# microsoft/fadtk

Measured on AMD Instinct MI355X. Metric: FAD scores/sec + cov-GEMM TFLOP/s (% MFMA peak), N=100k D=512, higher is better.
Workload: dtype f16 in, f16 MFMA with f32 accumulate over <= 8192-row runs, f64 across runs (moments); split-f16 MFMA iterations (f32 accumulate) + exact int8-MFMA products (int32 accumulate) + f64 correction (Frechet)

## Files before the change

### fadtk_amd/csrc/frechet.hip

```cpp
#include "frechet_internal.h"
#include "ns_mean.h"
#include "ns_fast.h"
#include "ns_fast_big.h"
#include "ns_fast_res.h"

#include <algorithm>
#include <atomic>
#include <cmath>
#include <type_traits>

namespace fad {

Pool& thread_pool(int device) {
    static thread_local PerThreadDevice<Pool> set;
    return set.get(device);
}
Workspace* free_slot(int device) {
    Pool& p = thread_pool(device);
    for (Workspace& w : p.slot)
        if (!w.busy) { w.pool = &p; return &w; }
    return nullptr;
}

SongKnobs SongKnobs::from_env() {
// ... 582 lines not shown
    int k = 1, upto = resident ? 1 : 9;
    for (;;) {
        for (; k < upto; ++k) {
            const int cur = k & 1;
            nsf::SplitArgs g = split_args();
            g.A[0] = Z[cur]; g.B[0] = Y[cur]; g.C[0] = T; g.alpha = -0.5f; g.beta_eye = 1.5f; g.gamma = 1.0f;
            g.partials = partials; g.skip = &s32_0->done; g.k = k;
            if (big) FAD_TRY(fast_split_big(d, nsf::SP_T, g, st, (unsigned)B, device));
            else fast_split(d, nsf::SP_T, g, st, (unsigned)B);
            g = split_args();
            g.A[0] = Y[cur]; g.B[0] = T; g.C[0] = Y[cur ^ 1]; g.A[1] = T; g.B[1] = Z[cur]; g.C[1] = Z[cur ^ 1];
            g.skip = &s32_0->upd_skip[k & 1];
            g.k = k; g.max_low = kMaxLow; g.nslots = big ? fast_big_t_slots(d, (unsigned)B) : nb * nb; g.chk_partials = partials; g.thr_pred = pred_threshold(ws.pool, d);
            if (big) FAD_TRY(fast_split_big(d, nsf::SP_U, g, st, (unsigned)B, device));
            else fast_split(d, nsf::SP_U, g, st, (unsigned)B);
        }
        if (!res_full) {
            nsf::DigArgs dg;
            memset(&dg, 0, sizeof(dg));
            dg.d = d; dg.gen = gen; dg.hA = hdr_b; dg.hB = reinterpret_cast<nsf::MatHdr*>(at(L.hdr)); dg.pstride = (int64_t)L.stride; dg.s32 = s32_0;
            dg.Y[0] = Y[0]; dg.Y[1] = Y[1]; dg.dig[0] = digY[0]; dg.dig[1] = digY[1]; dg.dig_t[0] = digYt[0]; dg.dig_t[1] = digYt[1];
            hipLaunchKernelGGL(nsf::nsf_digitize, dim3((unsigned)((dd / 16 + 255) / 256), 2, (unsigned)B), dim3(256), 0, st, dg);
        }
        if (!res_full) {
            nsf::I8Args a;
            memset(&a, 0, sizeof(a));
            a.Adig = digY[0]; a.Bdig = digYt[0]; a.Adig_alt = digY[1]; a.Bdig_alt = digYt[1]; a.sel = &s32_0->final_iter;
            a.d = d; a.gen = gen; a.hA = hdr_b; a.hB = reinterpret_cast<nsf::MatHdr*>(at(L.hdr)); a.pstride = (int64_t)L.stride; a.hstride = (int64_t)hs;
            a.skip = &s32_0->skip_corr; a.stats = h_stats; a.st = st0; a.A64in = A64;
            a.Y[0] = Y[0]; a.Y[1] = Y[1]; a.Z[0] = Z[0]; a.Z[1] = Z[1]; a.s32 = s32_0; a.host_words = h_words; a.host_vals = h_vals;
            for (int64_t b = 0; b < B; ++b) reinterpret_cast<int*>(reinterpret_cast<char*>(h_words) + b * hs)[12] = 0;
            if (big && d >= 256) FAD_TRY(fast_i8_big(d, nsf::I8_G, a, st, (unsigned)B, device));
            else fast_i8(d, nsf::I8_G, a, st, (unsigned)B);
        }
        FAD_HIP_TRY(hipGetLastError());
        FAD_HIP_TRY(hipStreamSynchronize(st));
        bool pending = false;
        for (int64_t b = 0; b < B; ++b) {
            if (settled[b]) continue;
            const int* hw = reinterpret_cast<const int*>(reinterpret_cast<const char*>(h_words) + b * hs);
            const double* hv = reinterpret_cast<const double*>(reinterpret_cast<const char*>(h_vals) + b * hs);
            const double* hx = reinterpret_cast<const double*>(reinterpret_cast<const char*>(h_stats) + b * hs);
            if (hw[12] != gen) return set_error(FAD_ERR_HIP, "the correction kernel of the batched fast chain left no result for song %lld", (long long)b);
            MixedResult r;
            fast_decide_one(hw, hv, hx, nb, &r);
            if (r.status == 0 && k < kMaxLow && !resident) { pending = true; continue; }
            settled[b] = 1;
            if (r.status == 1) { ok[b] = 1; tr_sqrt[b] = std::sqrt(r.c) * r.tr_scaled; }
            if (trace)
                fprintf(stderr, "[fad fast songs] song %lld: status %d iters %d decided_at %d res %.3e est %.3e tr %.6e c %.3e (words bad %d done %d ok %d failed %d skipped %d)\n",
                        (long long)b, r.status, r.iters, r.decided_at, r.res, r.est, r.tr_scaled, r.c, hw[0], hw[1], hw[5], hw[6], hw[11]);
            if (trace && b == 0) {
                fprintf(stderr, "[fad fast songs] song 0 residuals:");
                for (int q = 1; q < 16 && q <= r.iters; ++q) fprintf(stderr, " %.3e", hv[4 + q]);
                fprintf(stderr, "\n");
            }
        }
        if (!pending) break;
        upto = kMaxLow;
    }
    return FAD_OK;
}


struct PairBlock {
    size_t hdrA, hdrB, st, s32, partials, stats, A64, P, Y[2], Z[2], T, digA, digB, digY[2], digYt[2], mus, covs, Rv, Pv, Ev, stride;
};
static PairBlock pair_block(int d) {
    const size_t dd = (size_t)d * d, nb = (size_t)d / 32;
    PairBlock b; size_t o = 0;
    auto take = [&](size_t bytes) { const size_t at = o; o += (bytes + 255) & ~(size_t)255; return at; };
    b.hdrA = take(sizeof(nsf::MatHdr)); b.hdrB = take(sizeof(nsf::MatHdr)); b.st = take(sizeof(NsState)); b.s32 = take(sizeof(Ns32State));
    b.partials = take(nb * nb * sizeof(double)); b.stats = take(nsf::kTileStats * nb * nb * sizeof(double));
    b.A64 = take(8 * dd); b.P = take(8 * dd);
    b.Y[0] = take(8 * dd); b.Y[1] = take(8 * dd); b.Z[0] = take(8 * dd); b.Z[1] = take(8 * dd); b.T = take(8 * dd);
    b.digA = take(6 * dd); b.digB = take(6 * dd);
    b.digY[0] = take(6 * dd); b.digYt[0] = take(6 * dd); b.digY[1] = take(6 * dd); b.digYt[1] = take(6 * dd);
    b.mus = take(2 * (size_t)d * sizeof(double)); b.covs = take(2 * dd * sizeof(double));
    b.Rv = take(8 * dd); b.Pv = take(8 * dd); b.Ev = take(8 * dd);
    b.stride = o;
    return b;
}

static int pairs_verify_enqueue(Workspace& ws, int d, int B, hipStream_t st) {
    const size_t dd = (size_t)d * d;
    const PairBlock L = pair_block(d);
    const size_t hs = song_host_stride(d);
    char* blk = static_cast<char*>(ws.fast_pairs.p);
    char* hpin = static_cast<char*>(ws.fast_pairs_pin);
    auto at = [&](size_t off) { return blk + off; };
    auto mat = [&](size_t off) { nsf::SplitMat m; m.a = reinterpret_cast<uint4*>(at(off)); m.at = reinterpret_cast<uint4*>(at(off + 4 * dd)); return m; };
    nsf::SplitArgs g;
    memset(&g, 0, sizeof(g));
    g.d = d; g.gen = ws.multi.gen; g.hA = reinterpret_cast<nsf::MatHdr*>(at(L.hdrA)); g.hB = reinterpret_cast<nsf::MatHdr*>(at(L.hdrB));
    g.pstride = (int64_t)L.stride; g.astride = (int64_t)L.stride;
    g.st = reinterpret_cast<NsState*>(at(L.st)); g.s32 = reinterpret_cast<Ns32State*>(at(L.s32));
    const nsf::SplitMat Y[2] = {mat(L.Y[0]), mat(L.Y[1])}, Z[2] = {mat(L.Z[0]), mat(L.Z[1])};
    const int nb = d / 32;
    int* h_words = reinterpret_cast<int*>(hpin + (nsf::kHostVals + (size_t)(nsf::kTileStats + 2) * nb * nb) * sizeof(double));
    double* h_vstats = reinterpret_cast<double*>(hpin + host_vstats_off(d));
    for (int b = 0; b < B; ++b) reinterpret_cast<int*>(reinterpret_cast<char*>(h_words) + (size_t)b * hs)[13] = 0;
    fast_verify_launch(d, (unsigned)B, g, Y, Z, mat(L.Rv), mat(L.Pv), mat(L.Ev), g.s32, h_vstats, h_words, (int64_t)hs, st);
    FAD_HIP_TRY(hipGetLastError());
    FAD_HIP_TRY(hipEventRecord(ws.done_ev, st));
    return FAD_OK;
}

static int pairs_enqueue(Workspace& ws, int d, int B, const fad_moments_t* const* h1, const fad_moments_t* const* h2, int ddof,
                         int mean_dtype, hipStream_t st) {
    const size_t dd = (size_t)d * d;
    const int nb = d / 32;
    constexpr int kPairsBigMin = 3;
    const bool big = B >= kPairsBigMin && d >= 256;
    const bool wide = wide_enabled(ws.pool);
    const int max_low = wide ? kMaxLowWide : kMaxLow;
    const int device = ws.job.device;
    const PairBlock L = pair_block(d);
    const size_t hs = song_host_stride(d);
    void* const before = ws.fast_pairs.p;
    FAD_TRY(ws.fast_pairs.reserve((size_t)(B > 16 ? kMaxMultiPairs : B > 8 ? 16 : B > 4 ? 8 : 4) * L.stride + 256));
    if (!ws.fast_pairs_pin || ws.fast_pairs_pin_cap < (size_t)B * hs) {
        if (ws.fast_pairs_pin) (void)hipHostFree(ws.fast_pairs_pin);
        ws.fast_pairs_pin = nullptr; ws.fast_pairs_pin_cap = 0;
        FAD_HIP_TRY(hipHostMalloc(&ws.fast_pairs_pin, (size_t)kMaxMultiPairs * hs + 4096, hipHostMallocDefault));
        ws.fast_pairs_pin_cap = (size_t)kMaxMultiPairs * hs + 4096;
    }
    char* blk = static_cast<char*>(ws.fast_pairs.p);
    char* hpin = static_cast<char*>(ws.fast_pairs_pin);
    double* h_vals = reinterpret_cast<double*>(hpin);
    double* h_stats = h_vals + nsf::kHostVals;
    int* h_words = reinterpret_cast<int*>(h_stats + (size_t)(nsf::kTileStats + 2) * nb * nb);
    auto at = [&](size_t off) { return blk + off; };
    auto mat = [&](size_t off) { nsf::SplitMat m; m.a = reinterpret_cast<uint4*>(at(off)); m.at = reinterpret_cast<uint4*>(at(off + 4 * dd)); return m; };
    const int gen = ++ws.fast_gen;
    if (ws.fast_gen > (1 << 30)) ws.fast_gen = 1;
    ws.multi.gen = gen;
    if (ws.fast_pairs.p != before) {
        FAD_HIP_TRY(hipMemset2DAsync(at(L.hdrA), L.stride, 0, sizeof(nsf::MatHdr), (size_t)B, st));
        FAD_HIP_TRY(hipMemset2DAsync(at(L.hdrB), L.stride, 0, sizeof(nsf::MatHdr), (size_t)B, st));
    }
    nsf::MatHdr* hA = reinterpret_cast<nsf::MatHdr*>(at(L.hdrA));
    nsf::MatHdr* hB = reinterpret_cast<nsf::MatHdr*>(at(L.hdrB));
    NsState* st0 = reinterpret_cast<NsState*>(at(L.st));
    Ns32State* s32_0 = reinterpret_cast<Ns32State*>(at(L.s32));
    double* partials = reinterpret_cast<double*>(at(L.partials));
    double* stats = reinterpret_cast<double*>(at(L.stats));
    double* A64 = reinterpret_cast<double*>(at(L.A64));
    const nsf::SplitMat P = mat(L.P), Y[2] = {mat(L.Y[0]), mat(L.Y[1])}, Z[2] = {mat(L.Z[0]), mat(L.Z[1])}, T = mat(L.T);
    uint4* digY[2] = {reinterpret_cast<uint4*>(at(L.digY[0])), reinterpret_cast<uint4*>(at(L.digY[1]))};
    uint4* digYt[2] = {reinterpret_cast<uint4*>(at(L.digYt[0])), reinterpret_cast<uint4*>(at(L.digYt[1]))};

    static_assert(2 * kMaxMultiPairs <= nsf::kPrepMaxSets, "PrepArgs holds two sets per pair of a batch");
    nsf::PrepArgs pa;
    memset(&pa, 0, sizeof(pa));
    for (int b = 0; b < B; ++b) {
        pa.accs[2 * b] = moments_packed(h1[b]); pa.accs[2 * b + 1] = moments_packed(h2[b]);
        pa.runs[2 * b] = moments_runsum(h1[b]); pa.runs[2 * b + 1] = moments_runsum(h2[b]);
    }
    pa.acc[0] = pa.accs[0]; pa.acc[1] = pa.accs[1];
    pa.d = d; pa.ddof = ddof; pa.gen = gen; pa.mean_dtype = mean_dtype;
    pa.mus = reinterpret_cast<double*>(at(L.mus)); pa.covs = reinterpret_cast<double*>(at(L.covs));
    pa.dig[0] = reinterpret_cast<uint4*>(at(L.digA)); pa.dig[1] = reinterpret_cast<uint4*>(at(L.digB));
    pa.st = st0; pa.hdr[0] = hA; pa.hdr[1] = hB;
    pa.batch = 2; pa.pstride = (int64_t)L.stride; pa.no_covs = 1;
    pa.per = ((dd / 2048) % 4 == 0) ? 4 : 2;
    hipLaunchKernelGGL(nsf::nsf_prepare, dim3((unsigned)(dd / 2048 / pa.per + 1), (unsigned)(2 * B)), dim3(512), 0, st, pa);

    auto split_args = [&]() {
        nsf::SplitArgs g;
        memset(&g, 0, sizeof(g));
        g.d = d; g.gen = gen; g.hA = hA; g.hB = hB; g.pstride = (int64_t)L.stride; g.astride = (int64_t)L.stride;
        g.st = st0; g.s32 = s32_0;
        if (wide) { g.scaled = 1; g.lp_wide = 1; g.l0_scale = kWideL0Scale; g.l0_min = kWideL0Min; }
        return g;
    };
    {
        nsf::I8Args a;
        memset(&a, 0, sizeof(a));
        a.Adig = reinterpret_cast<uint4*>(at(L.digA)); a.Bdig = reinterpret_cast<uint4*>(at(L.digB)); a.d = d; a.gen = gen; a.hA = hA; a.hB = hB;
        a.pstride = (int64_t)L.stride; a.astride = (int64_t)L.stride; a.stats = stats; a.A64 = A64; a.P = P; a.st = st0;
        if (big) FAD_TRY(fast_i8_big(d, nsf::I8_A, a, st, (unsigned)B, device));
        else fast_i8(d, nsf::I8_A, a, st, (unsigned)B);
        nsf::SplitArgs g = split_args();
        g.A[0] = P; g.B[0] = P; g.C[0] = Y[1]; g.C[1] = Z[1]; g.A64 = A64; g.statsA = stats;
        if (big) FAD_TRY(fast_split_big(d, nsf::SP_FIRST, g, st, (unsigned)B, device));
        else { g.Cdig[0] = digY[1]; g.Cdig_t[0] = digYt[1]; fast_split(d, nsf::SP_FIRST, g, st, (unsigned)B); }
    }
    int want = ws.pool ? ws.pool->lp_iters : 5;
    if (want < 2) want = 2;
    if (want > max_low) want = max_low;
    for (int k = 1; k < want; ++k) {
        const int cur = k & 1;
        nsf::SplitArgs g = split_args();
        g.A[0] = Z[cur]; g.B[0] = Y[cur]; g.C[0] = T; g.alpha = -0.5f; g.beta_eye = 1.5f; g.gamma = 1.0f;
        g.partials = partials; g.skip = &s32_0->done; g.k = k;
        if (big) FAD_TRY(fast_split_big(d, nsf::SP_T, g, st, (unsigned)B, device));
        else fast_split(d, nsf::SP_T, g, st, (unsigned)B);
        g = split_args();
        g.A[0] = Y[cur]; g.B[0] = T; g.C[0] = Y[cur ^ 1]; g.A[1] = T; g.B[1] = Z[cur]; g.C[1] = Z[cur ^ 1];
        if (!big) { g.Cdig[0] = digY[cur ^ 1]; g.Cdig_t[0] = digYt[cur ^ 1]; }
        g.skip = &s32_0->upd_skip[k & 1];
        g.k = k; g.max_low = max_low; g.nslots = big ? fast_big_t_slots(d, (unsigned)B) : nb * nb; g.chk_partials = partials; g.thr_pred = pred_threshold(ws.pool, d);
        if (big) FAD_TRY(fast_split_big(d, nsf::SP_U, g, st, (unsigned)B, device));
        else fast_split(d, nsf::SP_U, g, st, (unsigned)B);
    }
    if (big) {
        nsf::DigArgs dg;
        memset(&dg, 0, sizeof(dg));
        dg.d = d; dg.gen = gen; dg.hA = hA; dg.hB = hB; dg.pstride = (int64_t)L.stride; dg.astride = (int64_t)L.stride; dg.s32 = s32_0;
        dg.Y[0] = Y[0]; dg.Y[1] = Y[1]; dg.dig[0] = digY[0]; dg.dig[1] = digY[1]; dg.dig_t[0] = digYt[0]; dg.dig_t[1] = digYt[1];
        hipLaunchKernelGGL(nsf::nsf_digitize, dim3((unsigned)((dd / 16 + 255) / 256), 2, (unsigned)B), dim3(256), 0, st, dg);
    }
    {
        nsf::I8Args a;
        memset(&a, 0, sizeof(a));
        a.Adig = digY[0]; a.Bdig = digYt[0]; a.Adig_alt = digY[1]; a.Bdig_alt = digYt[1]; a.sel = &s32_0->final_iter;
        a.d = d; a.gen = gen; a.hA = hA; a.hB = hB; a.pstride = (int64_t)L.stride; a.astride = (int64_t)L.stride; a.hstride = (int64_t)hs;
        a.skip = &s32_0->skip_corr; a.stats = h_stats; a.st = st0; a.A64in = A64;
        a.Y[0] = Y[0]; a.Y[1] = Y[1]; a.Z[0] = Z[0]; a.Z[1] = Z[1]; a.s32 = s32_0; a.host_words = h_words; a.host_vals = h_vals;
        if (wide) { a.Rv = mat(L.Rv); a.scaled = 1; }
        for (int b = 0; b < B; ++b) { int* w = reinterpret_cast<int*>(reinterpret_cast<char*>(h_words) + (size_t)b * hs); w[12] = 0; w[13] = 0; }
        if (big) FAD_TRY(fast_i8_big(d, nsf::I8_G, a, st, (unsigned)B, device));
        else fast_i8(d, nsf::I8_G, a, st, (unsigned)B);
    }
    FAD_HIP_TRY(hipGetLastError());
    if (!ws.done_ev) FAD_HIP_TRY(hipEventCreateWithFlags(&ws.done_ev, hipEventDisableTiming));
    if (wide && ws.pool && ws.pool->lp_verify) return pairs_verify_enqueue(ws, d, B, st);
    FAD_HIP_TRY(hipEventRecord(ws.done_ev, st));
    return FAD_OK;
}

static int mixed_begin(const NsProblem& pb, int device, hipStream_t stream, Workspace& ws) {
    const int d = pb.d;
    const int64_t dd = (int64_t)d * d;
    FAD_TRY(ws.mats.reserve((size_t)(6 * dd) * sizeof(double)));
    FAD_TRY(ws.mats32.reserve((size_t)(5 * dd) * sizeof(float)));
    const size_t hbytes = ws.job.fast ? fast_pinned_bytes(d) : sizeof(NsState) + sizeof(MixedResult);
    if (!ws.pinned || ws.pinned_cap < hbytes) {
        if (ws.pinned) (void)hipHostFree(ws.pinned);
        ws.pinned = nullptr; ws.pinned_cap = 0;
        FAD_HIP_TRY(hipHostMalloc(&ws.pinned, hbytes + 4096, hipHostMallocDefault));
        ws.pinned_cap = hbytes + 4096;
    }
    MixedBufs m = mixed_bufs(ws, d);
    m.hres->status = -1;
    ws.job.d = d; ws.job.device = device; ws.job.stream = stream; ws.job.k = 0;
    if (ws.job.fast) {
        ws.job.mu1 = pb.mu1; ws.job.mu2 = pb.mu2; ws.job.mean_dtype = pb.mean_dtype;
        int want = ws.pool ? ws.pool->lp_iters : 5;
        if (want < 2) want = 2;
        if (want > max_low_of(ws)) want = max_low_of(ws);
        if (ws.pool && ws.pool->lp_hopeless) want = 1;
        return fast_enqueue(ws, want);
    }
    NsProductExt ext;
    memset(&ext, 0, sizeof(ext));
    ext.stats = m.tilestats; ext.mu1 = pb.mu1; ext.mu2 = pb.mu2; ext.mean_dtype = pb.mean_dtype; ext.st = m.dstate;
    FAD_TRY(gemm_f64_product_stats_launch(d, pb.cov1, pb.cov2, m.A, &m.dstate->done, ext, stream));
    enqueue_ns_prepare(m.tilestats, d, (int)m.nb, pb.mu1, 0, pb.mu2, 0, pb.mean_dtype, m.dstate, 1, m.s32, 1, stream);
    int want = ws.pool ? ws.pool->lp_iters : 5;
    if (want < 2) want = 2;
    if (want > kMaxLow) want = kMaxLow;
    return mixed_enqueue(ws, want);
}

static int mixed_finish(Workspace& ws, MixedResult* res) {
    MixedBufs m = mixed_bufs(ws, ws.job.d);
    const int max_low = max_low_of(ws);
    bool asked = false;
    for (;;) {
        FAD_HIP_TRY(hipEventSynchronize(ws.done_ev));
        if (ws.job.fast) FAD_TRY(fast_decide(ws));
        if (m.hres->status == 5) {
            if (asked) { m.hres->status = 2; break; }
            asked = true;
            FAD_TRY(fast_verify_enqueue(ws));
            continue;
        }
        if (m.hres->status == 4) {
            ws.job.k = m.hres->iters;
            m.hres->status = 0;
        } else if (m.hres->status != 0 || ws.job.k >= max_low) {
            break;
        }
        if (ws.job.k >= max_low) break;
        const int step = (ws.job.fast && max_low > kMaxLow) ? 4 : 2;
        const int upto = (ws.job.k + step < max_low) ? ws.job.k + step : max_low;
        FAD_TRY(ws.job.fast ? fast_enqueue(ws, upto) : mixed_enqueue(ws, upto));
    }
    *res = *m.hres;
    if (res->status == 0) res->status = 2;
    if (res->status == 1 && res->decided_at >= 0 && ws.pool) ws.pool->lp_iters = res->decided_at + 1;
    if (ws.pool && ws.job.fast) {
        ws.pool->lp_hopeless = res->status == 2 && res->iters < 0;
        ws.pool->lp_verify = res->status == 1 && res->pad == 1;
    }
    return FAD_OK;
}

static bool mixed_eligible(Workspace& ws, int d, int max_iter, double tol) {
    Pool* p = ws.pool;
    if (p && p->mixed < 0) { const char* e = getenv("FAD_FRECHET_MIXED"); p->mixed = (e && e[0] == '0') ? 0 : 1; }
    return (!p || p->mixed) && d % 64 == 0 && max_iter <= 0 && tol <= 0.0;
}

static int frechet_single(int d, const double* cov1, const double* cov2, const double* mu1, const double* mu2,
                          double eps, int max_iter, double tol, int mean_dtype, int device, hipStream_t stream,
// ... 188 lines not shown
        if (moments_dim(h1[b]) != d || moments_dim(h2[b]) != d)
            return set_error(FAD_ERR_SHAPE, "Training and test covariances have different dimensions (pair %d: %d vs %d, pair 0: %d)", b,
                             moments_dim(h1[b]), moments_dim(h2[b]), d);
        if (moments_device(h1[b]) != device || moments_device(h2[b]) != device) return set_error(FAD_ERR_INVALID, "handles live on different devices");
    }
    DeviceGuard g(device);
    hipStream_t st = static_cast<hipStream_t>(stream);
    Workspace* wsp = free_slot(device);
    if (!wsp) return set_error(FAD_ERR_INVALID, "all %d Frechet slots of this thread are in flight: collect one with fad_frechet_end", Pool::kSlots);
    Workspace& ws = *wsp;
    ws.pool = &thread_pool(device);
    ws.job = Workspace::Job();
    ws.job.d = d; ws.job.device = device; ws.job.stream = st; ws.job.eps = eps; ws.job.mean_dtype = mean_dtype; ws.job.ddof = ddof;
    ws.multi = Workspace::Multi();
    ws.multi.count = count;
    for (int b = 0; b < count; ++b) { ws.multi.h1[b] = h1[b]; ws.multi.h2[b] = h2[b]; }
    if (fast_eligible(ws, d, 0, 0.0)) {
        for (int b = 0; b < count; ++b) { FAD_TRY(moments_settle(h1[b], st)); FAD_TRY(moments_settle(h2[b], st)); }
        FAD_TRY(pairs_enqueue(ws, d, count, h1, h2, ddof, mean_dtype, st));
        for (int b = 0; b < count; ++b) { FAD_TRY(moments_mark_read(h1[b], st)); FAD_TRY(moments_mark_read(h2[b], st)); }
        ws.multi.enqueued = true;
    }
    ws.busy = true;
    *job = reinterpret_cast<fad_frechet_job_t*>(wsp);
    return FAD_OK;
}

int fad_frechet_multi_end(fad_frechet_job_t* job, int count, double* out_fad, fad_diag_t* diag) {
    if (!job || !out_fad) return set_error(FAD_ERR_INVALID, "NULL argument");
    Workspace& ws = *reinterpret_cast<Workspace*>(job);
    if (!ws.busy) return set_error(FAD_ERR_INVALID, "this job was collected already");
    if (count != ws.multi.count) return set_error(FAD_ERR_INVALID, "this job holds %d pairs, not %d", ws.multi.count, count);
    const Workspace::Job j = ws.job;
    const Workspace::Multi m = ws.multi;
    DeviceGuard g(j.device);
    const int d = j.d, nb = d / 32;
    bool done[kMaxMultiPairs] = {false};
    int chain_status[kMaxMultiPairs];
    for (int b = 0; b < kMaxMultiPairs; ++b) chain_status[b] = -1;
    int rc = FAD_OK;
    if (m.enqueued) {
        const hipError_t e = hipEventSynchronize(ws.done_ev);
        if (e != hipSuccess) { ws.busy = false; return set_error(FAD_ERR_HIP, "hipEventSynchronize failed: %s", hipGetErrorString(e)); }
        const size_t hs = song_host_stride(d);
        const char* hpin = static_cast<const char*>(ws.fast_pairs_pin);
        const size_t off_stats = nsf::kHostVals * sizeof(double), off_words = off_stats + (size_t)(nsf::kTileStats + 2) * nb * nb * sizeof(double);
        const size_t off_vstats = host_vstats_off(d);
        const bool wide = wide_enabled(ws.pool);
        int learnt = -1;
        bool any_verified = false;
        for (int round = 0; round < 2; ++round) {
            bool ask = false;
            for (int b = 0; b < count; ++b) {
                if (done[b]) continue;
                const double* hv = reinterpret_cast<const double*>(hpin + (size_t)b * hs);
                const double* hx = reinterpret_cast<const double*>(hpin + (size_t)b * hs + off_stats);
                const int* hw = reinterpret_cast<const int*>(hpin + (size_t)b * hs + off_words);
                const double* hvx = reinterpret_cast<const double*>(hpin + (size_t)b * hs + off_vstats);
                if (hw[12] != m.gen) continue;
                MixedResult r;
                fast_decide_one(hw, hv, hx, nb, &r, wide ? hvx : nullptr, m.gen, wide ? kMaxLowWide : kMaxLow);
                chain_status[b] = r.status;
                if (r.too_few0 || r.too_few1) {
                    if (rc == FAD_OK) rc = set_error(FAD_ERR_TOO_FEW_ROWS, "FAD requires at least two embedding window frames in each set");
                    out_fad[b] = NAN; done[b] = true;
                    continue;
                }
                if (r.status == 5 && round == 0) { ask = true; continue; }
                if (r.status != 1) continue;
                const double tr_sqrt = sqrt(r.c) * r.tr_scaled;
                out_fad[b] = r.mean_term + r.tr1 + r.tr2 - 2.0 * tr_sqrt;
                if (diag) {
                    fad_diag_t& q = diag[b];
                    memset(&q, 0, sizeof(q));
                    q.iters = r.iters + 1; q.converged = 3; q.used_eps = 0; q.route = 2;
                    q.residual = r.res; q.scale = r.c; q.mean_term = r.mean_term; q.tr1 = r.tr1; q.tr2 = r.tr2; q.tr_sqrt = tr_sqrt;
                    q.verified = r.pad == 1 ? 1 : 0;
                }
                if (r.decided_at + 1 > learnt) learnt = r.decided_at + 1;
                if (r.pad == 1) any_verified = true;
                done[b] = true;
            }
            if (!ask) break;
            const int rv = pairs_verify_enqueue(ws, d, count, j.stream);
            if (rv != FAD_OK) { if (rc == FAD_OK) rc = rv; break; }
            const hipError_t e2 = hipEventSynchronize(ws.done_ev);
            if (e2 != hipSuccess) { ws.busy = false; return set_error(FAD_ERR_HIP, "hipEventSynchronize failed: %s", hipGetErrorString(e2)); }
        }
        if (learnt > 0 && ws.pool) ws.pool->lp_iters = learnt;
        if (ws.pool && wide) ws.pool->lp_verify = any_verified;

        int declined = 0;
        for (int b = 0; b < count; ++b) if (!done[b] && chain_status[b] == 2) ++declined;
        if (rc == FAD_OK && declined >= 2) {
            const PairBlock L = pair_block(d);
            const size_t dd = (size_t)d * d;
            char* blk = static_cast<char*>(ws.fast_pairs.p);
            const int64_t stride = (int64_t)(L.stride / sizeof(double));
            const double* mus = reinterpret_cast<const double*>(blk + L.mus);
            const double* covs = reinterpret_cast<const double*>(blk + L.covs);
            int r2 = ws.small.reserve(ns_small_bytes(d, count));
            NsState* hst = nullptr;
            if (r2 == FAD_OK) {
                NsState* dstates = static_cast<NsState*>(ws.small.p);
                enqueue_clear_states(dstates, count, j.stream);
                uint32_t mask = 0;
                for (int b = 0; b < count; ++b) if (done[b] || chain_status[b] != 2) mask |= (1u << b);
                if (mask) enqueue_mark_states_done(dstates, mask, count, j.stream);
                nsf::PrepArgs pc;
                memset(&pc, 0, sizeof(pc));
                for (int b = 0; b < count; ++b) { pc.accs[2 * b] = moments_packed(m.h1[b]); pc.accs[2 * b + 1] = moments_packed(m.h2[b]); }
                pc.d = d; pc.ddof = j.ddof; pc.batch = 2; pc.pstride = (int64_t)L.stride;
                pc.covs = reinterpret_cast<double*>(blk + L.covs);
                hipLaunchKernelGGL(nsf::nsf_pairs_covs, dim3((unsigned)(dd / 2048), (unsigned)(2 * count)), dim3(512), 0, j.stream, pc);
                NsProblem pb{d, count, covs, stride, covs + dd, stride, mus, stride, mus + d, stride, j.mean_dtype};
                r2 = run_ns(pb, 0, 0.0, j.device, j.stream, ws, &hst, false, nullptr, (ws.pool && ws.pool->f64_iters_multi > 0) ? ws.pool->f64_iters_multi + 1 : 0);
            }
            if (r2 == FAD_OK && hst) {
                int most = 0;
                for (int b = 0; b < count; ++b) {
                    if (done[b] || chain_status[b] != 2) continue;
                    const NsState& q = hst[b];
                    if (q.nonfinite || q.conv == 0 || !q.finished || q.final_iter < 0) continue;
                    const double tr_sqrt = sqrt(q.c) * q.tr_last;
                    out_fad[b] = q.mean_term + q.tr1 + q.tr2 - 2.0 * tr_sqrt;
                    if (diag) {
                        fad_diag_t& g2 = diag[b];
                        memset(&g2, 0, sizeof(g2));
                        g2.iters = q.final_iter + 1; g2.converged = q.conv; g2.used_eps = 0; g2.route = 0; g2.residual = q.res_last;
                        g2.scale = q.c; g2.mean_term = q.mean_term; g2.tr1 = q.tr1; g2.tr2 = q.tr2; g2.tr_sqrt = tr_sqrt;
                    }
                    if (q.final_iter + 1 > most) most = q.final_iter + 1;
                    done[b] = true;
                }
                if (most > 0 && ws.pool) ws.pool->f64_iters_multi = most;
            }
        }
    }
    ws.busy = false;
    ws.multi = Workspace::Multi();
    for (int b = 0; b < count; ++b) {
        if (done[b]) continue;
        const int r1 = fad_frechet_from_moments(m.h1[b], m.h2[b], j.ddof, j.eps, 0, 0.0, j.mean_dtype, j.stream, &out_fad[b], diag ? &diag[b] : nullptr);
        if (r1 != FAD_OK && rc == FAD_OK) rc = r1;
    }
    return rc;
}

int fad_frechet_cancel(fad_frechet_job_t* job) {
    if (!job) return set_error(FAD_ERR_INVALID, "NULL argument");
    Workspace& ws = *reinterpret_cast<Workspace*>(job);
    if (!ws.busy) return FAD_OK;
    DeviceGuard g(ws.job.device);
    if ((ws.job.mixed || ws.multi.enqueued) && ws.done_ev) FAD_HIP_TRY(hipEventSynchronize(ws.done_ev));
    else FAD_HIP_TRY(hipStreamSynchronize(ws.job.stream));
    ws.busy = false;
    ws.job = Workspace::Job();
    ws.multi = Workspace::Multi();
    return FAD_OK;
}

}
```

### fadtk_amd/csrc/frechet_internal.h

```cpp
#pragma once
#include "fad_common.h"
#include "ns_check.h"
#include "ns32.h"

#include <cstdlib>
#include <vector>

struct fad_moments;
namespace fad {
const double* moments_packed(const fad_moments* h);
int moments_settle(const fad_moments* h, hipStream_t st);
int moments_mark_read(const fad_moments* h, hipStream_t st);
int moments_device(const fad_moments* h);
int moments_dim(const fad_moments* h);
const float* moments_runsum(const fad_moments* h);

constexpr int kStatScal = 8;
static inline int64_t stat_blocks(int d) { return cdiv(d, 32); }
static inline size_t stat_doubles(int d) { const int64_t nb = stat_blocks(d); return (size_t)(2 * nb * d + kStatScal * nb * nb); }

constexpr int kMaxMultiPairs = 32;

struct Workspace : NsWorkspace {
    DevBuf rows, offs, songbuf, songmat, rows2, songrun, songjobs;
    DevBuf base_root;
    void* song_pin = nullptr; size_t song_pin_cap = 0;
    DevBuf mats32;
    DevBuf fast;
    int fast_gen = 0;
    DevBuf songcov;
    DevBuf fast_songs;
    void* fast_songs_pin = nullptr; size_t fast_songs_pin_cap = 0;
    DevBuf fast_pairs;
    void* fast_pairs_pin = nullptr; size_t fast_pairs_pin_cap = 0;
    struct Multi {
        int count = 0, gen = 0;
        bool enqueued = false;
        const fad_moments_t* h1[kMaxMultiPairs] = {nullptr}; const fad_moments_t* h2[kMaxMultiPairs] = {nullptr};
    } multi;
    bool busy = false;
    struct Job {
        int d = 0, device = 0, k = 0, mean_dtype = -1, ddof = 1;
        bool mixed = false;
        bool fast = false;
        int gen = 0;
        double eps = 0.0;
        hipStream_t stream = nullptr;
        const double *cov1 = nullptr, *cov2 = nullptr, *mu1 = nullptr, *mu2 = nullptr;
    } job;
    hipEvent_t done_ev = nullptr;
    struct Pool* pool = nullptr;
    void release_all() {
        release(); rows.release(); offs.release(); songbuf.release(); songmat.release(); rows2.release(); songrun.release(); songjobs.release(); mats32.release(); base_root.release(); fast.release();
        fast_songs.release(); songcov.release(); fast_pairs.release();
        if (fast_pairs_pin) { (void)hipHostFree(fast_pairs_pin); fast_pairs_pin = nullptr; fast_pairs_pin_cap = 0; }
        if (fast_songs_pin) { (void)hipHostFree(fast_songs_pin); fast_songs_pin = nullptr; fast_songs_pin_cap = 0; }
        if (done_ev) { (void)hipEventDestroy(done_ev); done_ev = nullptr; }
        if (song_pin) { (void)hipHostFree(song_pin); song_pin = nullptr; song_pin_cap = 0; }
    }
    int reserve_song_pin(size_t bytes) {
        if (song_pin && song_pin_cap >= bytes) return FAD_OK;
        if (song_pin) (void)hipHostFree(song_pin);
        song_pin = nullptr; song_pin_cap = 0;
        FAD_HIP_TRY(hipHostMalloc(&song_pin, bytes + bytes / 2 + 4096, hipHostMallocDefault));
        song_pin_cap = bytes + bytes / 2 + 4096;
        return FAD_OK;
    }
};


struct Pool {
    static constexpr int kSlots = 8;
    Workspace slot[kSlots];
    int lp_iters = 5;
    bool lp_hopeless = false;
    bool lp_verify = false;
    int lp_wide = -1;
    int f64_iters = 0;
    int f64_iters_multi = 0;
    int mixed = -1;
    int fast = -1;
    double pred_thr = 0.0;
    void release_all() { for (Workspace& w : slot) w.release_all(); }
};
Pool& thread_pool(int device);
Workspace* free_slot(int device);

struct NsProblem {
    int d; int64_t B;
    const double* cov1; int64_t s_cov1;
    const double* cov2; int64_t s_cov2;
    const double* mu1; int64_t s_mu1;
    const double* mu2; int64_t s_mu2;
    int mean_dtype;
    int sym = 0;
};

static inline int ns_pstride(int d) {
    const int64_t a = gemm_f64_slots_max(d), b = cdiv((int64_t)d * d, 256);
    return (int)(a > b ? a : b);
}
static inline size_t ns_small_bytes(int d, int64_t B) {
    return (size_t)B * (sizeof(NsState) + sizeof(Ns32State) + ((size_t)ns_pstride(d) + stat_doubles(d)) * sizeof(double)) + 256;
}

__device__ __forceinline__ void sum_partials(const double* __restrict__ rowabs, const double* __restrict__ colabs, int nb,
                                             int d, int i, double& rs, double& cs) {
    rs = 0.0; cs = 0.0;
    int k = 0;
    for (; k + 8 <= nb; k += 8) {
        double r[8], c[8];
#pragma unroll
        for (int q = 0; q < 8; ++q) { r[q] = rowabs[(int64_t)(k + q) * d + i]; c[q] = colabs[(int64_t)(k + q) * d + i]; }
#pragma unroll
        for (int q = 0; q < 8; ++q) { rs += r[q]; cs += c[q]; }
    }
    for (; k < nb; ++k) { rs += rowabs[(int64_t)k * d + i]; cs += colabs[(int64_t)k * d + i]; }
}

constexpr int kSymMaxIter = 16;
// ... 27 lines not shown
```

### fadtk_amd/csrc/ns_fast.h

```cpp
#pragma once
#include "fad_common.h"
#include "ns_check.h"
#include "ns32.h"
#include "ns_mean.h"

namespace fad {
namespace nsf {

typedef int i32x4 __attribute__((ext_vector_type(4)));
typedef int i32x16 __attribute__((ext_vector_type(16)));
typedef _Float16 f16x8 __attribute__((ext_vector_type(8)));
typedef _Float16 f16x2 __attribute__((ext_vector_type(2)));

constexpr int kDigits = 6;
constexpr int kUminA = 3, kUminG = 4;
constexpr float kLoScale = 2048.f, kLoInv = 1.f / 2048.f;
constexpr int kTileStats = 4;

__device__ __host__ __forceinline__ size_t fa_idx(int rb, int ks, int plane, int lane, int d) {
    return (((size_t)rb * (size_t)(d >> 4) + (size_t)ks) * 2 + (size_t)plane) * 64 + (size_t)lane;
}
__device__ __host__ __forceinline__ size_t dg_idx(int rb, int ks, int p, int lane, int d) {
    return (((size_t)rb * (size_t)(d >> 5) + (size_t)ks) * kDigits + (size_t)p) * 64 + (size_t)lane;
}
// ... 20 lines not shown
    hi = (_Float16)v;
    lo = (_Float16)((v - (float)hi) * kLoScale);
}
__device__ __forceinline__ float used16(_Float16 hi, _Float16 lo) { return (float)hi + (float)lo * kLoInv; }

template <int N, int NW = 8> __device__ __forceinline__ void wg8_sum(double (&v)[N], double* red) {
#pragma unroll
    for (int q = 0; q < N; ++q)
#pragma unroll
        for (int off = 32; off > 0; off >>= 1) v[q] += __shfl_xor(v[q], off);
    __syncthreads();
    if ((threadIdx.x & 63) == 0) {
#pragma unroll
        for (int q = 0; q < N; ++q) red[(threadIdx.x >> 6) * N + q] = v[q];
    }
    __syncthreads();
#pragma unroll
    for (int q = 0; q < N; ++q) {
        double t = 0.0;
#pragma unroll
        for (int w = 0; w < NW; ++w) t += red[w * N + q];
        v[q] = t;
    }
}
template <int NW = 8> __device__ __forceinline__ double wg8_max(double v, double* red) {
#pragma unroll
    for (int off = 32; off > 0; off >>= 1) v = fmax(v, __shfl_xor(v, off));
    __syncthreads();
    if ((threadIdx.x & 63) == 0) red[threadIdx.x >> 6] = v;
    __syncthreads();
    double t = red[0];
#pragma unroll
    for (int w = 1; w < NW; ++w) t = fmax(t, red[w]);
    return t;
}

__device__ __forceinline__ void tile_of_block(int& ty, int& tx) {
    ty = blockIdx.y; tx = blockIdx.x;
    const int t = gridDim.x;
    if ((t & 3) == 0) {
        const int b = blockIdx.y * t + blockIdx.x;
        const int xcd = b & 7, idx = b >> 3;
        const int R = t >> 1, Cc = t >> 2;
        ty = (xcd >> 2) * R + idx / Cc;
        tx = (xcd & 3) * Cc + idx % Cc;
    }
}

struct MatHdr {
    double s;
    double tr;
    int bad;
    int flag_gen;
    int pad[2];
};
__device__ __forceinline__ bool hdr_bad(const MatHdr* a, const MatHdr* b, int gen) {
    return (a->bad | b->bad) != 0 || a->flag_gen == gen || b->flag_gen == gen;
}
__device__ __forceinline__ double hdr_inv_s12(const MatHdr* a, const MatHdr* b) { return 1.0 / (a->s * b->s); }

template <class T> __device__ __forceinline__ T* adv(T* p, int64_t bytes) {
    return reinterpret_cast<T*>(reinterpret_cast<uintptr_t>(p) + (uintptr_t)bytes);
}

struct SplitMat { uint4* a; uint4* at; };
__device__ __forceinline__ SplitMat adv(const SplitMat& m, int64_t bytes) { return SplitMat{adv(m.a, bytes), adv(m.at, bytes)}; }

constexpr int kPrepMaxSets = 64;
struct PrepArgs {
    const double* acc[2];
    const double* cov_in[2];
    const double* mu_in[2];
    int d, ddof, gen, mean_dtype;
    double* mus;
    double* covs;
    uint4* dig[2];
    NsState* st; MatHdr* hdr[2];
    int batch; int64_t pstride;
    const double* accs[kPrepMaxSets];
    const float* run[2]; const float* runs[kPrepMaxSets];
    int no_covs;
    int per;
};

__device__ __forceinline__ double prep_cov(double m, double sr, double sk, double inv_n, double inv_nd) { return (m - (sr * sk) * inv_n) * inv_nd; }

__global__ __launch_bounds__(512) void nsf_prepare(PrepArgs a) {
    __shared__ double red[8 * 2];
    __shared__ double mu_lds[2 * 1024];
    __shared__ float gaps[1024];
    const int tid = threadIdx.x, d = a.d;
    const bool pairs = a.batch == 2, songs = a.batch == 1;
    const int set = songs ? (blockIdx.y ? 1 : 0) : (pairs ? (int)(blockIdx.y & 1) : (int)blockIdx.y);
    const int64_t po = songs ? (blockIdx.y ? (int64_t)(blockIdx.y - 1) * a.pstride : 0) : (pairs ? (int64_t)(blockIdx.y >> 1) * a.pstride : 0);
    if (!songs && blockIdx.x == gridDim.x - 1) {
        if (set != 0 || tid >= 256) return;
        double* mus = adv(a.mus, po);
        for (int q = 0; q < 2; ++q) {
            const double* acq = pairs ? a.accs[(blockIdx.y & ~1u) + q] : a.acc[q];
            const float* rq = pairs ? a.runs[(blockIdx.y & ~1u) + q] : a.run[q];
            for (int i = tid; i < d; i += 256) {
                const double m = acq ? ((rq ? numpy_mean_of_f32_sum(rq[i], acq[0]) : acq[1 + i] / acq[0])) : a.mu_in[q][i];
                mu_lds[q * 1024 + i] = m;
                if (acq) mus[(int64_t)q * d + i] = m;
            }
        }
        __syncthreads();
        const double mt = mean_term_block(mu_lds, mu_lds + 1024, d, a.mean_dtype, gaps, red);
        if (tid == 0) adv(a.st, po)->mean_term = mt;
        return;
    }
    const double* acc = pairs ? a.accs[blockIdx.y] : a.acc[set];
    const double n = acc ? acc[0] : 2.0;
    const double* sum = acc ? acc + 1 : nullptr;
    const double* M = acc ? acc + 1 + d : a.cov_in[set] + ((songs && blockIdx.y) ? (int64_t)(blockIdx.y - 1) * d * d : 0);
    MatHdr* hdr = adv(a.hdr[set], po);
    NsState* st = adv(a.st, po);
    const double inv_n = 1.0 / n, inv_nd = 1.0 / (n - (double)a.ddof);
    const int per = a.per > 1 ? a.per : 1;
    int T = blockIdx.x * per * 512 + tid;
    int qd = T & 3, piece = T >> 2;
    int r = piece & 31, g = (piece >> 5) & 1, ksrb = piece >> 6, ks = ksrb % (d >> 5), rb = ksrb / (d >> 5);
    int row = 32 * rb + r, k0 = 32 * ks + 16 * g + 4 * qd;
    double m[4], sk[4], sr = 0.0;
    const bool transposed = !acc && set == 1;
    auto fetch = [&]() {
        const double* Mrow = M + (int64_t)row * d + k0;
#pragma unroll
        for (int q = 0; q < 4; ++q) m[q] = transposed ? M[(int64_t)(k0 + q) * d + row] : Mrow[q];
        if (acc) {
            sr = sum[row];
#pragma unroll
            for (int q = 0; q < 4; ++q) sk[q] = sum[k0 + q];
        }
    };
    fetch();
    double tr1[1] = {0.0}, mx = 0.0;
    for (int i = tid; i < d; i += 512) {
        const double md = M[(int64_t)i * d + i];
        const double v = acc ? (md - (sum[i] * sum[i]) * inv_n) * inv_nd : md;
        tr1[0] += v; mx = fmax(mx, v);
    }
    mx = wg8_max(mx, red);
    wg8_sum<1>(tr1, red);
    const double tr = tr1[0];
    const bool few = acc && n < 2.0;
    const bool bad = few || !(tr == tr) || isinf(tr) || !(mx > 0.0) || isinf(mx);
    int ex = 0;
    if (!bad) (void)frexp(mx, &ex);
    const double s = bad ? 1.0 : ldexp(1.0, -ex);
    if (blockIdx.x == 0 && tid == 0) {
        hdr->s = s; hdr->tr = tr; hdr->bad = bad ? 1 : 0;
        if (!songs) st->too_few[set] = few ? 1 : 0;
        if (songs ? set == 1 : set == 0) {
            st->done = 0; st->finished = 0; st->nonfinite = 0; st->conv = 0; st->final_iter = -1;
            st->upd_skip[0] = 0; st->upd_skip[1] = 0;
            if (songs) { st->too_few[0] = 0; st->too_few[1] = 0; st->mean_term = 0.0; }
        }
    }
    bool off_grid = false;
    uint4* out = adv(a.dig[set], po);
    for (int it = 0; it < per; ++it) {
        if (it > 0) {
            T += 512;
            qd = T & 3; piece = T >> 2;
            r = piece & 31; g = (piece >> 5) & 1; ksrb = piece >> 6; ks = ksrb % (d >> 5); rb = ksrb / (d >> 5);
            row = 32 * rb + r; k0 = 32 * ks + 16 * g + 4 * qd;
            fetch();
        }
        uint32_t w[kDigits];
#pragma unroll
        for (int p = 0; p < kDigits; ++p) w[p] = 0u;
        double* cov_out = acc ? adv(a.covs, po) + (int64_t)set * d * d + (int64_t)row * d + k0 : nullptr;
#pragma unroll
        for (int q = 0; q < 4; ++q) {
            const double c0 = acc ? prep_cov(m[q], sr, sk[q], inv_n, inv_nd) : m[q];
            if (acc && !a.no_covs) cov_out[q] = c0;
            const double v = c0 * s;
            const bool fits = fabs(v) <= 1.9375;
            off_grid = off_grid || !fits;
            int dg[kDigits];
            digits_of<double>((bad || !fits) ? 0.0 : v, dg);
#pragma unroll
            for (int p = 0; p < kDigits; ++p) w[p] |= ((uint32_t)dg[p] & 0xffu) << (8 * q);
        }
#pragma unroll
        for (int p = 0; p < kDigits; ++p) reinterpret_cast<uint32_t*>(out + dg_idx(rb, ks, p, 32 * g + r, d))[qd] = w[p];
    }
    if (off_grid) hdr->flag_gen = a.gen;
}

__global__ __launch_bounds__(512) void nsf_pairs_covs(PrepArgs a) {
    const int d = a.d, set = (int)(blockIdx.y & 1);
    const int64_t po = (int64_t)(blockIdx.y >> 1) * a.pstride;
    const double* acc = a.accs[blockIdx.y];
    const double n = acc[0];
    const double* sum = acc + 1;
    const double* M = acc + 1 + d;
    const double inv_n = 1.0 / n, inv_nd = 1.0 / (n - (double)a.ddof);
    const int64_t e = ((int64_t)blockIdx.x * 512 + threadIdx.x) * 4;
    const int row = (int)(e / d), k0 = (int)(e - (int64_t)row * d);
    const double sr = sum[row];
    double* cov_out = adv(a.covs, po) + (int64_t)set * d * d + (int64_t)row * d + k0;
#pragma unroll
    for (int q = 0; q < 4; ++q) cov_out[q] = prep_cov(M[(int64_t)row * d + k0 + q], sr, sum[k0 + q], inv_n, inv_nd);
}

__device__ __forceinline__ void store_tile_planes(const float* fin, const SplitMat& X, int ty, int tx, int d, int tid) {
    {
        const bool tr = tid >= 128;
        const int ln = tid & 31, q = (tid >> 5) & 3;
        f16x8 hi, lo;
#pragma unroll
        for (int j = 0; j < 8; ++j) {
            const float v = tr ? fin[(8 * q + j) * 33 + ln] : fin[ln * 33 + 8 * q + j];
            _Float16 h, l; split16(v, h, l); hi[j] = h; lo[j] = l;
        }
        uint4* base = tr ? X.at : X.a;
        const int rb = tr ? tx : ty, ks = 2 * (tr ? ty : tx) + (q >> 1), lane = 32 * (q & 1) + ln;
        uint4 uh, ul; __builtin_memcpy(&uh, &hi, 16); __builtin_memcpy(&ul, &lo, 16);
        base[fa_idx(rb, ks, 0, lane, d)] = uh;
        base[fa_idx(rb, ks, 1, lane, d)] = ul;
    }
}
__device__ __forceinline__ void store_tile_digits(const float* fin, uint4* dig, uint4* dig_t, int ty, int tx, int d, int tid) {
    {
        const bool tr = tid < 256;
        const int u = tid & 255, ln = u & 31, q = u >> 5;
        uint32_t w[kDigits];
#pragma unroll
        for (int p = 0; p < kDigits; ++p) w[p] = 0u;
#pragma unroll
        for (int j = 0; j < 4; ++j) {
            const float v = tr ? fin[(4 * q + j) * 33 + ln] : fin[ln * 33 + 4 * q + j];
            _Float16 h, l; split16(v, h, l);
            int dg[kDigits];
            digits_of<float>(used16(h, l), dg);
#pragma unroll
            for (int p = 0; p < kDigits; ++p) w[p] |= ((uint32_t)dg[p] & 0xffu) << (8 * j);
        }
        uint4* base = tr ? dig_t : dig;
        const int rb = tr ? tx : ty, ks = tr ? ty : tx, lane = 32 * (q >> 2) + ln;
#pragma unroll
        for (int p = 0; p < kDigits; ++p)
            reinterpret_cast<uint32_t*>(base + dg_idx(rb, ks, p, lane, d))[q & 3] = w[p];
    }
}
__device__ __forceinline__ void store_tile(const float* fin, const SplitMat& X, uint4* dig, uint4* dig_t, int ty, int tx, int d, int tid) {
    if (tid < 256) store_tile_planes(fin, X, ty, tx, d, tid);
    if (dig) store_tile_digits(fin, dig, dig_t, ty, tx, d, tid);
}


enum { I8_A = 0, I8_G = 1 };
constexpr int kHostWords = 16, kHostVals = 24;
struct I8Args {
    const uint4* Adig; const uint4* Bdig;
    const uint4* Adig_alt; const uint4* Bdig_alt; const int* sel;
    int d, gen;
    const MatHdr* hA; const MatHdr* hB;
    int64_t pstride, hstride;
    int64_t astride;
    const int* skip;
    double* stats;
    double* A64; SplitMat P;
    NsState* st;
    const double* A64in;
    SplitMat Y[2], Z[2];
    const Ns32State* s32;
    int* host_words;
// ... 477 lines not shown
```

Measured before the change: 12550.

## Digitize only upper-triangle covariance tiles and defer verify correction launch

The pairs prepare kernel now processes only upper-triangular 32x32 tiles of each symmetric covariance. It computes the digits once and writes the transposed tile to the mirrored position through an LDS transpose, which roughly halves the global reads and digit computation. The int8 correction launch is moved into a helper. The extra Rv output it writes is now produced only when verification is enabled upfront, and otherwise it is recomputed later for unfinished pairs if verification is requested. This adds LDS traffic and syncthreads per iteration, plus a serial loop to locate each tile.

```diff
diff --git a/fadtk_amd/csrc/frechet.hip b/fadtk_amd/csrc/frechet.hip
--- a/fadtk_amd/csrc/frechet.hip
+++ b/fadtk_amd/csrc/frechet.hip
@@ -688,6 +688,8 @@
     return b;
 }
 
+constexpr int kPairsBigMin = 3;
+
 static int pairs_verify_enqueue(Workspace& ws, int d, int B, hipStream_t st) {
     const size_t dd = (size_t)d * d;
     const PairBlock L = pair_block(d);
@@ -712,11 +714,47 @@
     return FAD_OK;
 }
 
+static int pairs_corr_enqueue(Workspace& ws, int d, int B, bool with_rv, const bool* done, hipStream_t st) {
+    const size_t dd = (size_t)d * d;
+    const int nb = d / 32;
+    const bool big = B >= kPairsBigMin && d >= 256;
+    const bool wide = wide_enabled(ws.pool);
+    const PairBlock L = pair_block(d);
+    const size_t hs = song_host_stride(d);
+    char* blk = static_cast<char*>(ws.fast_pairs.p);
+    char* hpin = static_cast<char*>(ws.fast_pairs_pin);
+    double* h_vals = reinterpret_cast<double*>(hpin);
+    double* h_stats = h_vals + nsf::kHostVals;
+    int* h_words = reinterpret_cast<int*>(h_stats + (size_t)(nsf::kTileStats + 2) * nb * nb);
+    auto at = [&](size_t off) { return blk + off; };
+    auto mat = [&](size_t off) { nsf::SplitMat m; m.a = reinterpret_cast<uint4*>(at(off)); m.at = reinterpret_cast<uint4*>(at(off + 4 * dd)); return m; };
+    Ns32State* s32_0 = reinterpret_cast<Ns32State*>(at(L.s32));
+    nsf::I8Args a;
+    memset(&a, 0, sizeof(a));
+    a.Adig = reinterpret_cast<uint4*>(at(L.digY[0])); a.Bdig = reinterpret_cast<uint4*>(at(L.digYt[0]));
+    a.Adig_alt = reinterpret_cast<uint4*>(at(L.digY[1])); a.Bdig_alt = reinterpret_cast<uint4*>(at(L.digYt[1])); a.sel = &s32_0->final_iter;
+    a.d = d; a.gen = ws.multi.gen; a.hA = reinterpret_cast<nsf::MatHdr*>(at(L.hdrA)); a.hB = reinterpret_cast<nsf::MatHdr*>(at(L.hdrB));
+    a.pstride = (int64_t)L.stride; a.astride = (int64_t)L.stride; a.hstride = (int64_t)hs;
+    a.skip = &s32_0->skip_corr; a.stats = h_stats; a.st = reinterpret_cast<NsState*>(at(L.st)); a.A64in = reinterpret_cast<double*>(at(L.A64));
+    a.Y[0] = mat(L.Y[0]); a.Y[1] = mat(L.Y[1]); a.Z[0] = mat(L.Z[0]); a.Z[1] = mat(L.Z[1]); a.s32 = s32_0; a.host_words = h_words; a.host_vals = h_vals;
+    if (wide) a.scaled = 1;
+    if (with_rv) a.Rv = mat(L.Rv);
+    for (int b = 0; b < B; ++b) {
+        if (done && done[b]) {
+            FAD_HIP_TRY(hipMemsetD32Async(reinterpret_cast<hipDeviceptr_t>(at(L.s32 + (size_t)b * L.stride + offsetof(Ns32State, skip_corr))), 1, 1, st));
+            continue;
+        }
+        int* w = reinterpret_cast<int*>(reinterpret_cast<char*>(h_words) + (size_t)b * hs); w[12] = 0; w[13] = 0;
+    }
+    if (big) FAD_TRY(fast_i8_big(d, nsf::I8_G, a, st, (unsigned)B, ws.job.device));
+    else fast_i8(d, nsf::I8_G, a, st, (unsigned)B);
+    return FAD_OK;
+}
+
 static int pairs_enqueue(Workspace& ws, int d, int B, const fad_moments_t* const* h1, const fad_moments_t* const* h2, int ddof,
                          int mean_dtype, hipStream_t st) {
     const size_t dd = (size_t)d * d;
     const int nb = d / 32;
-    constexpr int kPairsBigMin = 3;
     const bool big = B >= kPairsBigMin && d >= 256;
     const bool wide = wide_enabled(ws.pool);
     const int max_low = wide ? kMaxLowWide : kMaxLow;
@@ -732,10 +770,6 @@
         ws.fast_pairs_pin_cap = (size_t)kMaxMultiPairs * hs + 4096;
     }
     char* blk = static_cast<char*>(ws.fast_pairs.p);
-    char* hpin = static_cast<char*>(ws.fast_pairs_pin);
-    double* h_vals = reinterpret_cast<double*>(hpin);
-    double* h_stats = h_vals + nsf::kHostVals;
-    int* h_words = reinterpret_cast<int*>(h_stats + (size_t)(nsf::kTileStats + 2) * nb * nb);
     auto at = [&](size_t off) { return blk + off; };
     auto mat = [&](size_t off) { nsf::SplitMat m; m.a = reinterpret_cast<uint4*>(at(off)); m.at = reinterpret_cast<uint4*>(at(off + 4 * dd)); return m; };
     const int gen = ++ws.fast_gen;
@@ -769,8 +803,8 @@
     pa.dig[0] = reinterpret_cast<uint4*>(at(L.digA)); pa.dig[1] = reinterpret_cast<uint4*>(at(L.digB));
     pa.st = st0; pa.hdr[0] = hA; pa.hdr[1] = hB;
     pa.batch = 2; pa.pstride = (int64_t)L.stride; pa.no_covs = 1;
-    pa.per = ((dd / 2048) % 4 == 0) ? 4 : 2;
-    hipLaunchKernelGGL(nsf::nsf_prepare, dim3((unsigned)(dd / 2048 / pa.per + 1), (unsigned)(2 * B)), dim3(512), 0, st, pa);
+    pa.per = 4;
+    hipLaunchKernelGGL(nsf::nsf_prepare, dim3((unsigned)nsf::prep_tri_grid(d, pa.per), (unsigned)(2 * B)), dim3(512), 0, st, pa);
 
     auto split_args = [&]() {
         nsf::SplitArgs g;
@@ -817,18 +851,9 @@
         dg.Y[0] = Y[0]; dg.Y[1] = Y[1]; dg.dig[0] = digY[0]; dg.dig[1] = digY[1]; dg.dig_t[0] = digYt[0]; dg.dig_t[1] = digYt[1];
         hipLaunchKernelGGL(nsf::nsf_digitize, dim3((unsigned)((dd / 16 + 255) / 256), 2, (unsigned)B), dim3(256), 0, st, dg);
     }
-    {
-        nsf::I8Args a;
-        memset(&a, 0, sizeof(a));
-        a.Adig = digY[0]; a.Bdig = digYt[0]; a.Adig_alt = digY[1]; a.Bdig_alt = digYt[1]; a.sel = &s32_0->final_iter;
-        a.d = d; a.gen = gen; a.hA = hA; a.hB = hB; a.pstride = (int64_t)L.stride; a.astride = (int64_t)L.stride; a.hstride = (int64_t)hs;
-        a.skip = &s32_0->skip_corr; a.stats = h_stats; a.st = st0; a.A64in = A64;
-        a.Y[0] = Y[0]; a.Y[1] = Y[1]; a.Z[0] = Z[0]; a.Z[1] = Z[1]; a.s32 = s32_0; a.host_words = h_words; a.host_vals = h_vals;
-        if (wide) { a.Rv = mat(L.Rv); a.scaled = 1; }
-        for (int b = 0; b < B; ++b) { int* w = reinterpret_cast<int*>(reinterpret_cast<char*>(h_words) + (size_t)b * hs); w[12] = 0; w[13] = 0; }
-        if (big) FAD_TRY(fast_i8_big(d, nsf::I8_G, a, st, (unsigned)B, device));
-        else fast_i8(d, nsf::I8_G, a, st, (unsigned)B);
-    }
+    const bool with_rv = wide && ws.pool && ws.pool->lp_verify;
+    FAD_TRY(pairs_corr_enqueue(ws, d, B, with_rv, nullptr, st));
+    ws.multi.rv_written = with_rv;
     FAD_HIP_TRY(hipGetLastError());
     if (!ws.done_ev) FAD_HIP_TRY(hipEventCreateWithFlags(&ws.done_ev, hipEventDisableTiming));
     if (wide && ws.pool && ws.pool->lp_verify) return pairs_verify_enqueue(ws, d, B, st);
@@ -1183,7 +1208,13 @@
                 done[b] = true;
             }
             if (!ask) break;
-            const int rv = pairs_verify_enqueue(ws, d, count, j.stream);
+            int rv = FAD_OK;
+            if (!ws.multi.rv_written) {
+                rv = pairs_corr_enqueue(ws, d, count, true, done, j.stream);
+                if (rv == FAD_OK) { const hipError_t e1 = hipGetLastError(); if (e1 != hipSuccess) rv = set_error(FAD_ERR_HIP, "launch of the correction failed: %s", hipGetErrorString(e1)); }
+                ws.multi.rv_written = rv == FAD_OK;
+            }
+            if (rv == FAD_OK) rv = pairs_verify_enqueue(ws, d, count, j.stream);
             if (rv != FAD_OK) { if (rc == FAD_OK) rc = rv; break; }
             const hipError_t e2 = hipEventSynchronize(ws.done_ev);
             if (e2 != hipSuccess) { ws.busy = false; return set_error(FAD_ERR_HIP, "hipEventSynchronize failed: %s", hipGetErrorString(e2)); }
diff --git a/fadtk_amd/csrc/frechet_internal.h b/fadtk_amd/csrc/frechet_internal.h
--- a/fadtk_amd/csrc/frechet_internal.h
+++ b/fadtk_amd/csrc/frechet_internal.h
@@ -36,6 +36,7 @@
     struct Multi {
         int count = 0, gen = 0;
         bool enqueued = false;
+        bool rv_written = false;
         const fad_moments_t* h1[kMaxMultiPairs] = {nullptr}; const fad_moments_t* h2[kMaxMultiPairs] = {nullptr};
     } multi;
     bool busy = false;
diff --git a/fadtk_amd/csrc/ns_fast.h b/fadtk_amd/csrc/ns_fast.h
--- a/fadtk_amd/csrc/ns_fast.h
+++ b/fadtk_amd/csrc/ns_fast.h
@@ -126,6 +126,9 @@
     int no_covs;
     int per;
 };
+__host__ __device__ __forceinline__ int prep_tri_blocks(int d) { return (d >> 5) * ((d >> 5) + 1) / 2; }
+__host__ __device__ __forceinline__ int prep_tri_grid(int d, int per) { return (prep_tri_blocks(d) + 2 * per - 1) / (2 * per) + 1; }
+constexpr int kPrepTriPitch = 36, kPrepTriPlane = 32 * kPrepTriPitch;
 
 __device__ __forceinline__ double prep_cov(double m, double sr, double sk, double inv_n, double inv_nd) { return (m - (sr * sk) * inv_n) * inv_nd; }
 
@@ -162,16 +165,26 @@
     NsState* st = adv(a.st, po);
     const double inv_n = 1.0 / n, inv_nd = 1.0 / (n - (double)a.ddof);
     const int per = a.per > 1 ? a.per : 1;
-    int T = blockIdx.x * per * 512 + tid;
+    const bool tri = pairs && a.no_covs;
+    bool live = true, mirror = false;
+    int T = tri ? (tid & 255) : blockIdx.x * per * 512 + tid;
     int qd = T & 3, piece = T >> 2;
     int r = piece & 31, g = (piece >> 5) & 1, ksrb = piece >> 6, ks = ksrb % (d >> 5), rb = ksrb / (d >> 5);
+    auto locate_tri = [&](int it) {
+        const int t = (blockIdx.x * per + it) * 2 + (tid >> 8);
+        live = t < prep_tri_blocks(d);
+        int i = 0, rem = live ? t : 0;
+        while (rem >= (d >> 5) - i) { rem -= (d >> 5) - i; ++i; }
+        rb = i; ks = i + rem; mirror = live && rem > 0;
+    };
+    if (tri) locate_tri(0);
     int row = 32 * rb + r, k0 = 32 * ks + 16 * g + 4 * qd;
     double m[4], sk[4], sr = 0.0;
     const bool transposed = !acc && set == 1;
     auto fetch = [&]() {
         const double* Mrow = M + (int64_t)row * d + k0;
 #pragma unroll
-        for (int q = 0; q < 4; ++q) m[q] = transposed ? M[(int64_t)(k0 + q) * d + row] : Mrow[q];
+        for (int q = 0; q < 4; ++q) m[q] = (transposed || (tri && k0 + q < row)) ? M[(int64_t)(k0 + q) * d + row] : Mrow[q];
         if (acc) {
             sr = sum[row];
 #pragma unroll
@@ -206,9 +219,12 @@
     uint4* out = adv(a.dig[set], po);
     for (int it = 0; it < per; ++it) {
         if (it > 0) {
-            T += 512;
-            qd = T & 3; piece = T >> 2;
-            r = piece & 31; g = (piece >> 5) & 1; ksrb = piece >> 6; ks = ksrb % (d >> 5); rb = ksrb / (d >> 5);
+            if (tri) locate_tri(it);
+            else {
+                T += 512;
+                qd = T & 3; piece = T >> 2;
+                r = piece & 31; g = (piece >> 5) & 1; ksrb = piece >> 6; ks = ksrb % (d >> 5); rb = ksrb / (d >> 5);
+            }
             row = 32 * rb + r; k0 = 32 * ks + 16 * g + 4 * qd;
             fetch();
         }
@@ -228,8 +244,26 @@
 #pragma unroll
             for (int p = 0; p < kDigits; ++p) w[p] |= ((uint32_t)dg[p] & 0xffu) << (8 * q);
         }
-#pragma unroll
-        for (int p = 0; p < kDigits; ++p) reinterpret_cast<uint32_t*>(out + dg_idx(rb, ks, p, 32 * g + r, d))[qd] = w[p];
+        if (live) {
+#pragma unroll
+            for (int p = 0; p < kDigits; ++p) reinterpret_cast<uint32_t*>(out + dg_idx(rb, ks, p, 32 * g + r, d))[qd] = w[p];
+        }
+        if (tri) {
+            unsigned char* tl = reinterpret_cast<unsigned char*>(mu_lds) + (tid >> 8) * (kDigits * kPrepTriPlane);
+            const int kl = 16 * g + 4 * qd;
+            if (it > 0) __syncthreads();
+#pragma unroll
+            for (int p = 0; p < kDigits; ++p)
+#pragma unroll
+                for (int q = 0; q < 4; ++q) tl[p * kPrepTriPlane + (kl + q) * kPrepTriPitch + r] = (unsigned char)(w[p] >> (8 * q));
+            __syncthreads();
+            if (mirror) {
+#pragma unroll
+                for (int p = 0; p < kDigits; ++p)
+                    reinterpret_cast<uint32_t*>(out + dg_idx(ks, rb, p, 32 * g + r, d))[qd] =
+                        *reinterpret_cast<const uint32_t*>(tl + p * kPrepTriPlane + r * kPrepTriPitch + kl);
+            }
+        }
     }
     if (off_grid) hdr->flag_gen = a.gen;
 }
```

New measurement: 12120. 0.965x the previous value.
